# linkedin/spark-tfrecord

Measured on AMD Instinct MI355X. Metric: rows/sec read+write (1M-row Example round-trip), higher is better.
Workload: dtype wire(int64/float32/bytes); 1 GPU; model=Example{id:int64, ints:Int64List[8], floats:FloatList[16], tokens:BytesList[2]}, global_batch=1000000, parallelism=dp1, rows_per_rank=1000000, engine=gpu, storage=/dev/shm, crc_verify=True

## Files before the change

csrc/hip/kernels.hip:

```cpp

#include <hip/hip_runtime.h>
#include <pybind11/pybind11.h>
#include <pybind11/stl.h>
#include <rocprim/rocprim.hpp>

#include <fcntl.h>
#include <sys/mman.h>
#include <sys/stat.h>
#include <unistd.h>

#include <cstdint>
#include <map>
#include <mutex>
#include <stdexcept>
#include <string>
#include <vector>

#include "../codec_core.h"

namespace py = pybind11;
using namespace tfrec;

#define HIP_CHECK(expr)                                                          \
  do {                                                                           \
// ... 68 lines not shown
        rc = scan_record(data, off[r], len[r], fmt, schema, st);
        payload_crc = crc32c_sw(data + off[r], (size_t)len[r], 0, tab);
      }
      if (rc != ERR_OK)
        payload_crc = crc32c_sw(data + off[r], (size_t)len[r], 0, tab);
      const u8* h = data + off[r] - 12;
      u32 len_crc, data_crc;
      __builtin_memcpy(&len_crc, h + 8, 4);
      __builtin_memcpy(&data_crc, h + 12 + len[r], 4);
      bool ok = mask_crc(crc32c_sw(h, 8, 0, tab)) == len_crc &&
                mask_crc(payload_crc) == data_crc;
      if (!ok) atomicMin(crc_err, (unsigned long long)(rec_base + r + 1));
    } else {
      rc = scan_record(data, off[r], len[r], fmt, schema, st);
    }
    if (rc != ERR_OK) set_err(err, rc, rec_base + r);
    for (int f = 0; f < F; ++f)
      if (st[f].err != ERR_OK) set_err(err, st[f].err, rec_base + r);
  }
}


struct DevFieldDst {
  int32_t kind;
  int32_t is_seq;
  i64* i64_vals;
  float* f32_vals;
  u8* bytes_data;
  i64* elem_len;
  i64* sub_count;
  const i64* val_base;
  const i64* byte_base;
  const i64* list_base;
};

__global__ void extract_fields_kernel(const u8* __restrict__ data, i64 R, int F,
                                      const FieldStat* __restrict__ stats,
                                      const DevFieldDst* __restrict__ metas,
                                      int32_t* __restrict__ err, i64 r0) {
  i64 total = R * F;
  for (i64 idx = blockIdx.x * (i64)blockDim.x + threadIdx.x; idx < total;
       idx += (i64)gridDim.x * blockDim.x) {
    i64 q = idx / F;
    int f = (int)(idx - q * F);
    i64 r = r0 + q;
    const DevFieldDst& m = metas[f];
    const FieldStat& st = stats[r * F + f];
    DecodeDst dst{m.i64_vals, m.f32_vals, m.bytes_data, m.elem_len, m.sub_count};
    int32_t rc = extract_field(data, st.pos, st.len, m.kind, m.is_seq, dst,
                               m.val_base ? m.val_base[r] : 0,
                               m.byte_base ? m.byte_base[r] : 0,
                               m.list_base ? m.list_base[r] : 0);
    if (rc != ERR_OK) set_err(err, rc, r);
  }
}



__global__ void size_records_kernel(const FieldColumn* __restrict__ cols,
                                    const u8* __restrict__ schema_blob, int32_t fmt,
                                    i64 R, i64* __restrict__ psize) {
  SchemaView schema = schema_view(schema_blob);
  for (i64 r = blockIdx.x * (i64)blockDim.x + threadIdx.x; r < R;
       r += (i64)gridDim.x * blockDim.x) {
    psize[r] = record_payload_size(cols, schema, fmt, r) + kFrameOverhead;
  }
}

__global__ void emit_records_kernel(const FieldColumn* __restrict__ cols,
                                    const u8* __restrict__ schema_blob, int32_t fmt,
                                    i64 r0, i64 R, const i64* __restrict__ frame_off,
                                    u8* __restrict__ file,
                                    int32_t* __restrict__ err) {
  __shared__ uint32_t tab[8][256];
  stage_crc_tables(tab);
  SchemaView schema = schema_view(schema_blob);
  for (i64 r = r0 + blockIdx.x * (i64)blockDim.x + threadIdx.x; r < R;
       r += (i64)gridDim.x * blockDim.x) {
    i64 payload = (frame_off[r + 1] - frame_off[r]) - kFrameOverhead;
    u8* o = file + frame_off[r] + 12;
// ... 289 lines not shown
      if (rc != ERR_OK) set_err(err, rc, rec_base + r);
      for (int f = 0; f < F; ++f)
        if (st[f].err != ERR_OK) set_err(err, st[f].err, rec_base + r);
    }
    if (crc_err) {
      const u8* h = data + off[r] - 12;
      u32 payload = crc32c_wave(h + 12, len[r], tab);
      if (lane == 0) {
        u32 len_crc, data_crc;
        __builtin_memcpy(&len_crc, h + 8, 4);
        __builtin_memcpy(&data_crc, h + 12 + len[r], 4);
        bool ok = mask_crc(crc32c_sw(h, 8, 0, tab)) == len_crc &&
                  mask_crc(payload) == data_crc;
        if (!ok) atomicMin(crc_err, (unsigned long long)(rec_base + r + 1));
      }
    }
  }
}

__global__ void extract_fields_wave_kernel(const u8* __restrict__ data, i64 R,
                                           int F,
                                           const FieldStat* __restrict__ stats,
                                           const DevFieldDst* __restrict__ metas,
                                           int32_t* __restrict__ err, i64 r0) {
  i64 total = R * F;
  i64 wave = (blockIdx.x * (i64)blockDim.x + threadIdx.x) / 64;
  i64 nwaves = ((i64)gridDim.x * blockDim.x) / 64;
  for (i64 idx = wave; idx < total; idx += nwaves) {
    i64 q = idx / F;
    int f = (int)(idx - q * F);
    i64 r = r0 + q;
    const DevFieldDst& m = metas[f];
    const FieldStat& st = stats[r * F + f];
    DecodeDst dst{m.i64_vals, m.f32_vals, m.bytes_data, m.elem_len, m.sub_count};
    int32_t rc = extract_field_wave(data, st.pos, st.len, m.kind, m.is_seq, dst,
                                    m.val_base ? m.val_base[r] : 0,
                                    m.byte_base ? m.byte_base[r] : 0,
                                    m.list_base ? m.list_base[r] : 0);
    if (rc != ERR_OK && (threadIdx.x & 63) == 0) set_err(err, rc, r);
  }
}


__device__ inline i64 wave_emit_i64_packed(u8* __restrict__ o,
                                           const i64* __restrict__ vals,
                                           i64 v0, i64 v1) {
  int lane = threadIdx.x & 63;
  i64 n = v1 - v0;
  i64 chunk = (n + 63) / 64;
  i64 lo = v0 + (i64)lane * chunk;
  i64 hi = lo + chunk < v1 ? lo + chunk : v1;
  i64 sz = 0;
  for (i64 v = lo; v < hi; ++v) sz += varint_size((u64)vals[v]);
  i64 incl = wave_incl_scan(sz);
  u8* q = o + (incl - sz);
  for (i64 v = lo; v < hi; ++v) q = write_varint(q, (u64)vals[v]);
  return __shfl(incl, 63);
}

struct WaveCur {
  u8* base;
  i64 pos;
};

__device__ inline void wvc_put(WaveCur& w, u8 b) {
  if ((threadIdx.x & 63) == 0) w.base[w.pos] = b;
// ... 251 lines not shown
    }
    if (threadIdx.x == 0) block_data[block_base + blockIdx.x] = (i64)cnt[0];
    return;
  }
  for (int off = 1; off < (int)blockDim.x; off <<= 1) {
    unsigned int v = (int)threadIdx.x >= off ? cnt[threadIdx.x - off] : 0;
    __syncthreads();
    cnt[threadIdx.x] += v;
    __syncthreads();
  }
  i64 slot = block_data[block_base + blockIdx.x] + (i64)(cnt[threadIdx.x] - my);
  if (c < c_hi)
    eval_frame_chunk(data, wdata, N, c, pos_start, pos_end, tab,
                     [&](i64 i, i64 len) {
                       cand_pos[slot] = i;
                       cand_len[slot] = len;
                       ++slot;
                     });
}

__global__ void frame_chain_kernel(const i64* __restrict__ pos,
                                   const i64* __restrict__ len, i64 C,
                                   const i64* __restrict__ carry_in,
                                   i64* __restrict__ carry_out,
                                   i64* __restrict__ off,
                                   i64* __restrict__ broken) {
  for (i64 k = blockIdx.x * (i64)blockDim.x + threadIdx.x; k < C;
       k += (i64)gridDim.x * blockDim.x) {
    i64 p = pos[k];
    i64 want = k == 0 ? *carry_in : pos[k - 1] + 16 + len[k - 1];
    if (p != want) *broken = 1;
    off[k] = p + 12;
    if (k == C - 1) *carry_out = p + 16 + len[k];
  }
}


struct InferSlot {
  unsigned long long hash;
  long long nameref;
  long long code;
};
static_assert(sizeof(InferSlot) == 24, "layout shared with Python [S,3] i64");

__device__ inline u64 fnv1a64(const u8* s, u64 n) {
  u64 h = 1469598103934665603ull;
  for (u64 i = 0; i < n; ++i) h = (h ^ s[i]) * 1099511628211ull;
  return h ? h : 1ull;
}

constexpr int kLdsInfer = 64;

struct LdsInferSlot {
  unsigned long long hash;
  long long nameref;
  unsigned int code;
};

__device__ inline bool lds_infer_merge(LdsInferSlot* ltab, u64 hash,
                                       long long nameref, int code) {
  int idx = (int)(hash % (u64)kLdsInfer);
  for (int probe = 0; probe < kLdsInfer; ++probe) {
    LdsInferSlot& s = ltab[idx];
    unsigned long long seen =
        atomicCAS(&s.hash, 0ull, (unsigned long long)hash);
    if (seen == 0ull) s.nameref = nameref;
// ... 220 lines not shown
                       dim3(kBlock), 0, (hipStream_t)stream, (const u8*)data,
                       (const i64*)off, (const i64*)len, R,
                       (unsigned long long*)err_out);
  } else {
    hipLaunchKernelGGL(crc_verify_kernel, dim3(grid_for(R)), dim3(kBlock), 0,
                       (hipStream_t)stream, (const u8*)data, (const i64*)off,
                       (const i64*)len, R, (unsigned long long*)err_out);
  }
  HIP_CHECK(hipGetLastError());
}

void gpu_scan_records(uintptr_t data, uintptr_t off, uintptr_t len, i64 R,
                      int32_t fmt, uintptr_t schema_blob, int F, uintptr_t stats,
                      uintptr_t err, uintptr_t crc_err, uintptr_t stream,
                      i64 avg_bytes, i64 rec_base, i64 max_blocks) {
  if (R <= 0) return;
  if (avg_bytes > kWaveRecordBytes) {
    hipLaunchKernelGGL(scan_records_wave_kernel,
                       dim3(grid_for(R * 64, max_blocks)), dim3(kBlock), 0,
                       (hipStream_t)stream, (const u8*)data, (const i64*)off,
                       (const i64*)len, R, fmt, (const u8*)schema_blob, F,
                       (FieldStat*)stats, (int32_t*)err,
                       (unsigned long long*)crc_err, rec_base);
  } else {
    hipLaunchKernelGGL(scan_records_kernel, dim3(grid_for(R, max_blocks)),
                       dim3(kBlock), 0, (hipStream_t)stream, (const u8*)data,
                       (const i64*)off, (const i64*)len, R, fmt,
                       (const u8*)schema_blob, F, (FieldStat*)stats,
                       (int32_t*)err, (unsigned long long*)crc_err, rec_base);
  }
  HIP_CHECK(hipGetLastError());
}

void gpu_extract_fields(uintptr_t data, i64 R, int F, uintptr_t stats,
                        py::list metas, uintptr_t meta_dev, uintptr_t err,
                        uintptr_t stream, i64 avg_bytes, i64 r0,
                        i64 max_blocks) {
  if (R <= 0 || F <= 0) return;
  std::vector<DevFieldDst> host_metas(F);
  for (int f = 0; f < F; ++f) {
    py::dict d = metas[f].cast<py::dict>();
    DevFieldDst& m = host_metas[f];
    m.kind = d["kind"].cast<int32_t>();
    m.is_seq = d["is_seq"].cast<int32_t>();
    m.i64_vals = (i64*)d["i64_vals"].cast<uintptr_t>();
    m.f32_vals = (float*)d["f32_vals"].cast<uintptr_t>();
    m.bytes_data = (u8*)d["bytes_data"].cast<uintptr_t>();
    m.elem_len = (i64*)d["elem_len"].cast<uintptr_t>();
    m.sub_count = (i64*)d["sub_count"].cast<uintptr_t>();
    m.val_base = (const i64*)d["val_base"].cast<uintptr_t>();
    m.byte_base = (const i64*)d["byte_base"].cast<uintptr_t>();
    m.list_base = (const i64*)d["list_base"].cast<uintptr_t>();
  }
  HIP_CHECK(hipMemcpyAsync((void*)meta_dev, host_metas.data(),
                           sizeof(DevFieldDst) * F, hipMemcpyHostToDevice,
                           (hipStream_t)stream));
  if (avg_bytes > kWaveRecordBytes) {
    hipLaunchKernelGGL(extract_fields_wave_kernel,
                       dim3(grid_for(R * F * 64, max_blocks)), dim3(kBlock), 0,
                       (hipStream_t)stream, (const u8*)data, R, F,
                       (const FieldStat*)stats, (const DevFieldDst*)meta_dev,
                       (int32_t*)err, r0);
  } else {
    hipLaunchKernelGGL(extract_fields_kernel,
                       dim3(grid_for(R * F, max_blocks)), dim3(kBlock), 0,
                       (hipStream_t)stream, (const u8*)data, R, F,
                       (const FieldStat*)stats, (const DevFieldDst*)meta_dev,
                       (int32_t*)err, r0);
  }
  HIP_CHECK(hipGetLastError());
}

size_t gpu_devcols_bytes(int F) { return sizeof(FieldColumn) * (size_t)F; }

void fill_devcols(py::list cols, std::vector<FieldColumn>& out) {
  int F = (int)cols.size();
  out.resize(F);
  for (int f = 0; f < F; ++f) {
    py::dict d = cols[f].cast<py::dict>();
    FieldColumn& c = out[f];
    c.kind = d["kind"].cast<int32_t>();
    c.is_seq = d["is_seq"].cast<int32_t>();
    c.presence = (const u8*)d["presence"].cast<uintptr_t>();
    c.row_off = (const i64*)d["row_off"].cast<uintptr_t>();
    c.list_off = (const i64*)d["list_off"].cast<uintptr_t>();
    c.sub_off = (const i64*)d["sub_off"].cast<uintptr_t>();
    c.elem_off = (const i64*)d["elem_off"].cast<uintptr_t>();
    c.bytes_data = (const u8*)d["values_bytes"].cast<uintptr_t>();
    c.i64_vals = (const i64*)d["values_i64"].cast<uintptr_t>();
// ... 58 lines not shown
void gpu_frame_scan_count(uintptr_t data, i64 N, i64 pos_start, i64 pos_end,
                          i64 block_base, uintptr_t block_counts,
                          uintptr_t stream) {
  i64 B = gpu_frame_scan_blocks(pos_start, pos_end);
  if (B <= 0) return;
  hipLaunchKernelGGL(frame_scan_pass_kernel<false>, dim3((uint32_t)B),
                     dim3(kBlock), 0, (hipStream_t)stream, (const u8*)data, N,
                     pos_start, pos_end, block_base, (i64*)block_counts,
                     nullptr, nullptr);
  HIP_CHECK(hipGetLastError());
}

void gpu_frame_scan_emit(uintptr_t data, i64 N, i64 pos_start, i64 pos_end,
                         i64 block_base, uintptr_t block_off,
                         uintptr_t cand_pos, uintptr_t cand_len,
                         uintptr_t stream) {
  i64 B = gpu_frame_scan_blocks(pos_start, pos_end);
  if (B <= 0) return;
  hipLaunchKernelGGL(frame_scan_pass_kernel<true>, dim3((uint32_t)B),
                     dim3(kBlock), 0, (hipStream_t)stream, (const u8*)data, N,
                     pos_start, pos_end, block_base, (i64*)block_off,
                     (i64*)cand_pos, (i64*)cand_len);
  HIP_CHECK(hipGetLastError());
}

void gpu_frame_chain(uintptr_t pos, uintptr_t len, i64 C, uintptr_t carry_in,
                     uintptr_t carry_out, uintptr_t off, uintptr_t broken,
                     uintptr_t stream) {
  if (C <= 0) return;
  hipLaunchKernelGGL(frame_chain_kernel, dim3(grid_for(C)), dim3(kBlock), 0,
                     (hipStream_t)stream, (const i64*)pos, (const i64*)len, C,
                     (const i64*)carry_in, (i64*)carry_out, (i64*)off,
                     (i64*)broken);
  HIP_CHECK(hipGetLastError());
}

void gpu_infer_codes(uintptr_t data, uintptr_t off, uintptr_t len, i64 R,
                     int32_t fmt, uintptr_t table, int nslots, uintptr_t err,
                     uintptr_t stream) {
  hipLaunchKernelGGL(infer_codes_kernel, dim3(grid_for(R)), dim3(kBlock), 0,
                     (hipStream_t)stream, (const u8*)data, (const i64*)off,
                     (const i64*)len, R, fmt, (InferSlot*)table, nslots,
                     (int32_t*)err);
  HIP_CHECK(hipGetLastError());
}

void gpu_gather_payloads(uintptr_t data, uintptr_t off, uintptr_t len,
                         uintptr_t dst_off, i64 R, uintptr_t out,
                         uintptr_t stream, i64 avg_bytes) {
  if (avg_bytes > kWaveRecordBytes) {
    hipLaunchKernelGGL(gather_payloads_wave_kernel, dim3(grid_for(R * 64)),
                       dim3(kBlock), 0, (hipStream_t)stream, (const u8*)data,
                       (const i64*)off, (const i64*)len, (const i64*)dst_off,
                       R, (u8*)out);
  } else {
    hipLaunchKernelGGL(gather_payloads_kernel, dim3(grid_for(R)), dim3(kBlock),
                       0, (hipStream_t)stream, (const u8*)data,
                       (const i64*)off, (const i64*)len, (const i64*)dst_off,
                       R, (u8*)out);
  }
  HIP_CHECK(hipGetLastError());
}


struct StridedLoadI64 {
  const i64* p;
// ... 252 lines not shown


void gpu_memcpy_d2h(uintptr_t dst, uintptr_t src, i64 n, uintptr_t stream) {
  HIP_CHECK(hipMemcpyAsync((void*)dst, (const void*)src, (size_t)n,
                           hipMemcpyDeviceToHost, (hipStream_t)stream));
}

void gpu_memcpy_h2d(uintptr_t dst, uintptr_t src, i64 n, uintptr_t stream) {
  HIP_CHECK(hipMemcpyAsync((void*)dst, (const void*)src, (size_t)n,
                           hipMemcpyHostToDevice, (hipStream_t)stream));
}

}

void register_gpu(py::module_& m) {
  m.def("gpu_device_count", []() {
    int n = 0;
    hipError_t e = hipGetDeviceCount(&n);
    return (e == hipSuccess) ? n : -static_cast<int>(e);
  });
  m.def("gpu_crc_verify", &gpu_crc_verify, py::arg("data"), py::arg("off"),
        py::arg("len"), py::arg("R"), py::arg("err_out"), py::arg("stream"),
        py::arg("avg_bytes") = 0);
  m.def("gpu_scan_records", &gpu_scan_records, py::arg("data"), py::arg("off"),
        py::arg("len"), py::arg("R"), py::arg("fmt"), py::arg("schema_blob"),
        py::arg("F"), py::arg("stats"), py::arg("err"), py::arg("crc_err"),
        py::arg("stream"), py::arg("avg_bytes") = 0, py::arg("rec_base") = 0,
        py::arg("max_blocks") = 0);
  m.def("gpu_extract_fields", &gpu_extract_fields, py::arg("data"),
        py::arg("R"), py::arg("F"), py::arg("stats"), py::arg("metas"),
        py::arg("meta_dev"), py::arg("err"), py::arg("stream"),
        py::arg("avg_bytes") = 0, py::arg("r0") = 0,
        py::arg("max_blocks") = 0);
  m.def("gpu_size_records", &gpu_size_records);
  m.def("gpu_emit_records", &gpu_emit_records, py::arg("cols_dev"),
        py::arg("schema_blob"), py::arg("fmt"), py::arg("r0"), py::arg("R"),
        py::arg("frame_off"), py::arg("file"), py::arg("err"),
        py::arg("stream"), py::arg("avg_bytes") = 0);
  m.def("gpu_frame_bytes", &gpu_frame_bytes, py::arg("src"),
        py::arg("elem_off"), py::arg("frame_off"), py::arg("R"),
        py::arg("file"), py::arg("stream"), py::arg("avg_bytes") = 0);
  m.def("gpu_frame_scan_blocks", &gpu_frame_scan_blocks);
  m.def("gpu_frame_scan_count", &gpu_frame_scan_count);
  m.def("gpu_frame_scan_emit", &gpu_frame_scan_emit);
  m.def("gpu_frame_chain", &gpu_frame_chain);
  m.def("gpu_gather_payloads", &gpu_gather_payloads, py::arg("data"),
        py::arg("off"), py::arg("len"), py::arg("dst_off"), py::arg("R"),
        py::arg("out"), py::arg("stream"), py::arg("avg_bytes") = 0);
  m.def("gpu_infer_codes", &gpu_infer_codes);
  m.def("gpu_scan_temp_bytes", &gpu_scan_temp_bytes);
  m.def("gpu_stat_scan_temp_bytes", &gpu_stat_scan_temp_bytes);
  m.def("gpu_stat_scans", &gpu_stat_scans, py::arg("temp"),
        py::arg("temp_bytes"), py::arg("stats"), py::arg("R"), py::arg("F"),
        py::arg("val_base"), py::arg("byte_base"), py::arg("list_base"),
        py::arg("stream"), py::arg("r0") = 0, py::arg("r1") = -1,
        py::arg("stride") = 0);
  m.def("gpu_excl_sum_strided", &gpu_excl_sum_strided);
  m.def("file_mmap_pinned", &file_mmap_pinned, py::arg("path"), py::arg("n"),
        py::arg("writable"));
  m.def("file_mmap_drop", &file_mmap_drop);
  m.def("file_mmap_sync", &file_mmap_sync);
  m.def("gpu_memcpy_d2h", &gpu_memcpy_d2h);
  m.def("gpu_memcpy_h2d", &gpu_memcpy_h2d);
  m.def("gpu_devcols_bytes", &gpu_devcols_bytes);
  m.def("gpu_devmeta_bytes", []() { return sizeof(DevFieldDst); });
  m.def("gpu_fieldstat_words", []() { return sizeof(FieldStat) / 8; });
}
```

spark_tfrecord_amd/engine/gpu.py:

```python

from __future__ import annotations

import os
from typing import List, Optional

import numpy as np
import torch

from .. import _native
from . import stream_plan
from ..columnar import RecordBatch, WireColumn, schema_blob, wire_fields
from ..schema import KIND_BYTES, KIND_FLOAT, KIND_INT64, StructType, is_sequence_field, wire_kind_of

FMT = {"Example": _native.FMT_EXAMPLE, "SequenceExample": _native.FMT_SEQUENCE}

_U64_MAX = 0xFFFFFFFFFFFFFFFF


def _stream() -> int:
    return torch.cuda.current_stream().cuda_stream


def _dev(x, dtype, device="cuda") -> torch.Tensor:
    if isinstance(x, torch.Tensor):
# ... 8 lines not shown

def check_native():
    if not getattr(_native, "HAS_GPU_KERNELS", False):
        raise RuntimeError("_native was built without HIP kernels; rebuild "
                           "with build_native.py before using the GPU engine")



import threading as _threading

_pinned_tls = _threading.local()


def pinned_buffer(tag: str, nbytes: int) -> torch.Tensor:
    pool = getattr(_pinned_tls, "pool", None)
    if pool is None:
        pool = _pinned_tls.pool = {}
    buf = pool.get(tag)
    if buf is None or buf.numel() < nbytes:
        cap = max(nbytes, int((buf.numel() if buf is not None else 1 << 20) * 1.5))
        buf = torch.empty(cap, dtype=torch.uint8, pin_memory=True)
        pool[tag] = buf
    return buf


_CHUNK = 64 << 20
_READ_SLICE = int(os.environ.get("TFREC_READ_SLICE", 32 << 20))
_SPLIT_SLICES = os.environ.get("TFREC_READ_SPLIT", "1") != "0"
_WRITE_SLICES = int(os.environ.get("TFREC_WRITE_SLICES", 8))
_STREAM_DECODE = os.environ.get("TFREC_STREAM_DECODE", "1") != "0"
_STREAM_HEADROOM = float(os.environ.get("TFREC_STREAM_HEADROOM", 1.125))
_STREAM_MAX_BLOCKS = int(os.environ.get("TFREC_STREAM_MAX_BLOCKS", 0))
_STREAM_EXTRACT = os.environ.get("TFREC_STREAM_EXTRACT", "1") != "0"
_SYNC_WRITES = os.environ.get("TFREC_SYNC", "1") != "0"


def read_file_to_device(path: str, device="cuda") -> torch.Tensor:
    import os as _os

    n = _os.path.getsize(path)
    dev_t = torch.empty(max(n, 1), dtype=torch.uint8, device=device)[:n]
    if n:
        ptr, pinned = _native.file_mmap_pinned(path, n, False)
        if pinned:
            _multi_dma(dev_t.data_ptr(), ptr, n, _native.gpu_memcpy_h2d,
                       after_main=True)
            return dev_t
    return _read_file_staged(path, dev_t)


_copy_streams: Optional[list] = None


def _dma_streams() -> list:
    global _copy_streams
    if _copy_streams is None:
        _copy_streams = [torch.cuda.Stream() for _ in range(2)]
    return _copy_streams


def _multi_dma(dst: int, src: int, n: int, fn, after_main: bool):
    streams = _dma_streams()
    main = torch.cuda.current_stream()
    k = min(len(streams), max(1, n // (16 << 20)))
    span = (n + k - 1) // k
    for i in range(k):
# ... 524 lines not shown
    data = torch.empty(n, dtype=torch.uint8, device=device)
    device = data.device
    plan = stream_plan.plan_slices(n, _READ_SLICE)
    S = len(plan)
    nblocks = [int(_native.gpu_frame_scan_blocks(p.scan_lo, p.scan_hi))
               if p.scan_hi > p.scan_lo else 0 for p in plan]
    block_counts = torch.empty(max(sum(nblocks), 1), dtype=torch.int64,
                               device=device)
    main = torch.cuda.current_stream()
    streams = _dma_streams()
    events = []
    for st in streams:
        st.wait_stream(main)
    for s, p in enumerate(plan):
        half = (p.b1 - p.b0) // 2 if _SPLIT_SLICES and len(streams) > 1 else 0
        parts = ([(p.b0, p.b0 + half, 0), (p.b0 + half, p.b1, 1)] if half
                 else [(p.b0, p.b1, s % len(streams))])
        evs = []
        for lo, hi, k in parts:
            st = streams[k]
            _native.gpu_memcpy_h2d(data.data_ptr() + lo, ptr + lo, hi - lo,
                                   st.cuda_stream)
            ev = torch.cuda.Event()
            ev.record(st)
            evs.append(ev)
        events.append(evs)
    data.record_stream(streams[0])
    if len(streams) > 1:
        data.record_stream(streams[1])

    fields = wire_fields(schema)
    F = len(fields)
    streaming = _STREAM_DECODE
    last_read.update(path="streamed", slices=S, regrows=0)
    do_scan = streaming and record_type != "ByteArray" and F > 0
    fuse_crc = verify_crc
    vals = None
    if streaming:
        status = torch.zeros(_ST_CARRY + 1 + S, dtype=torch.int64,
                             device=device)
        status[_ST_CRC] = -1
        sp = status.data_ptr()
        err = status[_ST_ERR:_ST_ERR + 1].view(torch.int32)
        xerr = status[_ST_XERR:_ST_XERR + 1].view(torch.int32)
        rows = _StreamRows(n, F if do_scan else 0, device)
        if do_scan:
            blob = _schema_blob_device(schema, device)
            vals = _StreamValues(fields, n, device) if _STREAM_EXTRACT else None
            meta_dev = torch.empty(F * _native.gpu_devmeta_bytes(),
                                   dtype=torch.uint8, device=device)

    base = 0
    C = 0
    nchain = 0
    r_done = 0
    pending = None
    avg_bytes = None
    for s, p in enumerate(plan):
        for ev in events[s]:
            main.wait_event(ev)
        last = s == S - 1
        nb = nblocks[s]
        if nb:
            _native.gpu_frame_scan_count(data.data_ptr(), n, p.scan_lo,
                                         p.scan_hi, base,
                                         block_counts.data_ptr(), _stream())
        if not streaming:
            base += nb
            continue
        if nb:
            block_off = excl_sum(block_counts[base:base + nb])
            c_s = int(block_off[-1].item())
            base += nb
            if c_s:
                rows.reserve(C + c_s, C, r_done, p.scan_hi)
                _native.gpu_frame_scan_emit(
                    data.data_ptr(), n, p.scan_lo, p.scan_hi, 0,
                    block_off.data_ptr(), rows.pos.data_ptr() + C * 8,
                    rows.lens.data_ptr() + C * 8, _stream())
                _native.gpu_frame_chain(
                    rows.pos.data_ptr() + C * 8, rows.lens.data_ptr() + C * 8,
                    c_s, sp + (_ST_CARRY + nchain) * 8,
                    sp + (_ST_CARRY + 1 + nchain) * 8,
                    rows.off.data_ptr() + C * 8, sp + _ST_BROKEN * 8, _stream())
                nchain += 1
                C += c_s
        if not do_scan or C == r_done:
            continue
        if last:
            avail = C
            end = n
        else:
            st_h = status.cpu()
            if int(st_h[_ST_BROKEN]) != 0:
                streaming = do_scan = False
                continue
            end = int(st_h[_ST_CARRY + nchain])
            avail = stream_plan.arrived_records(C, end, p.b1)
            if avail < C:
                end = p.b1
        if avail > r_done:
            if avg_bytes is None:
                avg_bytes = max(0, end // avail - 16)
            _native.gpu_scan_records(
                data.data_ptr(), rows.off.data_ptr() + r_done * 8,
                rows.lens.data_ptr() + r_done * 8, avail - r_done,
                FMT[record_type], blob.data_ptr(), F,
                rows.stats.data_ptr() + r_done * F * 48, err.data_ptr(),
                sp + _ST_CRC * 8 if fuse_crc else 0, _stream(), avg_bytes,
                rec_base=r_done, max_blocks=0 if last else _STREAM_MAX_BLOCKS)
            if vals is not None:
                rows.scan_stats(r_done, avail)
                if last:
                    pending = (r_done, avail)
                elif vals.ok:
                    h = torch.cat(rows.totals(avail)
                                  + [status[:_ST_CARRY]]).cpu()
                    pair = h[3 * F + _ST_ERR:3 * F + _ST_ERR + 1].view(torch.int32)
                    if int(h[3 * F + _ST_CRC]) != -1 or int(pair[0]) != 0:
                        vals.ok = False
                    else:
                        vals.extract(data, rows, r_done, avail,
                                     h[:3 * F].view(3, F), end, meta_dev,
                                     xerr, avg_bytes,
                                     _STREAM_MAX_BLOCKS)
            r_done = avail

    def unstreamed():
        last_read["path"] = "fallback" if _STREAM_DECODE else "unstreamed"
        ranges = [(p.scan_lo, p.scan_hi) for p in plan if p.scan_hi > p.scan_lo]
        off, lens, _ = _emit_and_chain(data, ranges, block_counts, n)
        return decode_device(data, off, lens, schema, record_type, verify_crc)

    if not streaming or C == 0:
        return unstreamed()
    R = C
    if not do_scan:
        st_h = status.cpu()
        if int(st_h[_ST_BROKEN]) != 0 or int(st_h[_ST_CARRY + nchain]) != n:
            return unstreamed()
        return decode_device(data, rows.off[:R], rows.lens[:R], schema,
                             record_type, verify_crc)

    stats = rows.stats[:R]
    if vals is None:
        rows.scan_stats(0, R)
    packed = torch.cat(rows.totals(R) + [status]).cpu()
    st_h = packed[3 * F:]
    if int(st_h[_ST_BROKEN]) != 0 or int(st_h[_ST_CARRY + nchain]) != n:
        return unstreamed()
    pair = st_h[_ST_ERR:_ST_ERR + 1].view(torch.int32)
    _raise_scan_errors(int(st_h[_ST_CRC]) if fuse_crc else -1, int(pair[0]),
                       int(pair[1]))
    totals_h = packed[:3 * F].view(3, F)
    val_base, byte_base, list_base = rows.planes
    if vals is None:
        cols = _extract_columns(data, R, fields, stats,
                                val_base[:, :R + 1], byte_base[:, :R + 1],
                                list_base[:, :R + 1], totals_h, xerr,
                                max(0, n // R - 16))
    else:
        if not vals.ok:
            raise RuntimeError("streamed decode: scan error lost")
        if pending is not None:
            vals.extract(data, rows, pending[0], pending[1], totals_h, n,
                         meta_dev, xerr, avg_bytes, 0)
        cols = vals.columns(stats, val_base, list_base, R)
    err_h = xerr.cpu()
    if int(err_h[0]) != 0:
        _raise_extract_error(int(err_h[0]), int(err_h[1]))
    return RecordBatch(schema, cols, R)


_ST_BROKEN, _ST_CRC, _ST_ERR, _ST_XERR, _ST_CARRY = 0, 1, 2, 3, 4


class _StreamRows:

    def __init__(self, total_bytes: int, F: int, device):
        self.total_bytes = total_bytes
        self.F = F
        self.device = device
        self.cap = 0
        self.pos = self.lens = self.off = self.stats = None
        self.planes = None

    def _alloc(self, cap: int):
        i64 = dict(dtype=torch.int64, device=self.device)
        planes = None
        if self.F:
            planes = [torch.empty((self.F, cap + 1), **i64) for _ in range(3)]
            for t in planes:
                t[:, 0] = 0
        return (torch.empty(cap, **i64), torch.empty(cap, **i64),
                torch.empty(cap, **i64),
                torch.empty((cap, self.F, 6), **i64) if self.F else None,
                planes)

    def scan_stats(self, r0: int, r1: int):
        ws = _stat_scan_workspace(r1 - r0, self.F, self.device)
        v, b, l = self.planes
        _native.gpu_stat_scans(ws.data_ptr(), ws.numel(),
                               self.stats.data_ptr(), r1, self.F, v.data_ptr(),
                               b.data_ptr(), l.data_ptr(), _stream(), r0=r0,
                               r1=r1, stride=self.cap + 1)

    def totals(self, r: int) -> list:
        return [t[:, r] for t in self.planes]

    def reserve(self, need: int, n_cand: int, n_scanned: int, bytes_seen: int):
        cap = stream_plan.grown_capacity(self.cap, need, bytes_seen,
                                         self.total_bytes, _STREAM_HEADROOM)
        if cap == self.cap:
            return
        pos, lens, off, stats, planes = self._alloc(cap)
        if n_cand:
            pos[:n_cand].copy_(self.pos[:n_cand])
            lens[:n_cand].copy_(self.lens[:n_cand])
            off[:n_cand].copy_(self.off[:n_cand])
        if n_scanned and stats is not None:
            stats[:n_scanned].copy_(self.stats[:n_scanned])
            for new, old in zip(planes, self.planes):
                new[:, :n_scanned + 1].copy_(old[:, :n_scanned + 1])
        self.pos, self.lens, self.off, self.stats = pos, lens, off, stats
        self.planes = planes
        if self.cap:
            last_read["regrows"] = last_read.get("regrows", 0) + 1
        self.cap = cap


class _StreamValues:

    _DIMS = (("i64_vals", 0), ("f32_vals", 0), ("elem_len", 0),
             ("bytes_data", 1), ("sub_count", 2))

    def __init__(self, fields, total_bytes: int, device):
        self.total_bytes = total_bytes
        self.device = device
        self.ok = True
        self.kinds = [wire_kind_of(f.dataType) for f in fields]
        self.seqs = [is_sequence_field(f.dataType) for f in fields]
        self.filled = [[0] * len(fields) for _ in range(3)]
        self.bufs = []
        for kind in self.kinds:
            dt = {"i64_vals": torch.int64, "f32_vals": torch.float32,
                  "elem_len": torch.int64, "bytes_data": torch.uint8,
                  "sub_count": torch.int64}
            self.bufs.append({k: torch.empty(0, dtype=d, device=device)
                              for k, d in dt.items()})

    def _used(self, i: int, name: str) -> bool:
        kind = self.kinds[i]
        return {"i64_vals": kind == KIND_INT64, "f32_vals": kind == KIND_FLOAT,
                "elem_len": kind == KIND_BYTES}.get(name, True)

    def _reserve(self, totals, bytes_seen: int):
        for i, bufs in enumerate(self.bufs):
            for name, dim in self._DIMS:
                if not self._used(i, name):
                    continue
                need = int(totals[dim][i])
                old = bufs[name]
                cap = stream_plan.grown_capacity(
                    old.numel(), need, bytes_seen, self.total_bytes,
                    _STREAM_HEADROOM, min_unit=1)
                if cap == old.numel():
                    continue
                new = torch.empty(cap, dtype=old.dtype, device=self.device)
                k = self.filled[dim][i]
                if k:
                    new[:k].copy_(old[:k])
                if old.numel():
                    last_read["regrows"] = last_read.get("regrows", 0) + 1
                bufs[name] = new

    def extract(self, data, rows, r0: int, r1: int, totals, bytes_seen: int,
                meta_dev, xerr, avg_bytes: int, max_blocks: int):
        self._reserve(totals, bytes_seen)
        v, b, l = rows.planes
        metas = []
        for i, bufs in enumerate(self.bufs):
            metas.append({
                "kind": self.kinds[i], "is_seq": 1 if self.seqs[i] else 0,
                "i64_vals": bufs["i64_vals"].data_ptr(),
                "f32_vals": bufs["f32_vals"].data_ptr(),
                "bytes_data": bufs["bytes_data"].data_ptr(),
                "elem_len": bufs["elem_len"].data_ptr(),
                "sub_count": bufs["sub_count"].data_ptr(),
                "val_base": v[i].data_ptr(),
                "byte_base": b[i].data_ptr(),
                "list_base": l[i].data_ptr() if self.seqs[i] else 0,
            })
        _native.gpu_extract_fields(data.data_ptr(), r1 - r0, len(self.bufs),
                                   rows.stats.data_ptr(), metas,
                                   meta_dev.data_ptr(), xerr.data_ptr(),
                                   _stream(), avg_bytes, r0=r0,
                                   max_blocks=max_blocks)
        self.filled = [[int(totals[d][i]) for i in range(len(self.bufs))]
                       for d in range(3)]

    def columns(self, stats, val_base, list_base, R: int) -> List[WireColumn]:
        cols = []
        for i, bufs in enumerate(self.bufs):
            kind, seq = self.kinds[i], self.seqs[i]
            nv, nb, nl = (self.filled[d][i] for d in range(3))
            presence = (stats[:, i, 0] >= 0).to(torch.uint8)
            elem_off = None
            if kind == KIND_BYTES:
                elem_off = excl_sum(bufs["elem_len"][:nv])
            sub_off = None
            if seq:
                sub_off = excl_sum(bufs["sub_count"][:nl])
            values = (bufs["i64_vals"][:nv] if kind == KIND_INT64 else
                      bufs["f32_vals"][:nv] if kind == KIND_FLOAT else
                      bufs["bytes_data"][:nb])
            cols.append(WireColumn(kind, seq, presence, val_base[i][:R + 1],
                                   values, elem_off,
                                   list_base[i][:R + 1] if seq else None,
                                   sub_off))
        return cols


def gz_device_meta(path: str):
    from ..io import paths as P

    if not getattr(_native, "HAS_GPU_KERNELS", False):
        return None
    return P.parse_gz_segments_file(path)


def _device_inflate_group(data: torch.Tensor, gz_items, device) -> bool:
    import os as _os

    comp_sizes = [_os.path.getsize(p) for p, _, _ in gz_items]
    comp_total = sum(comp_sizes)
    comp = torch.empty(max(comp_total, 1), dtype=torch.uint8,
                       device=device)[:comp_total]
    main = torch.cuda.current_stream()
    streams = _dma_streams()
    in_off = []
    in_len = []
    out_off = []
    out_len = []
    used = []
    coff = 0
    for k, (p, meta, out_base) in enumerate(gz_items):
        body_off, segs, _crc, _isize = meta
        ptr, pinned = _native.file_mmap_pinned(p, comp_sizes[k], False)
        if pinned:
            st = streams[k % len(streams)]
# ... 324 lines not shown
```

spark_tfrecord_amd/engine/stream_plan.py:

```python

from __future__ import annotations

from typing import List, NamedTuple

MIN_FRAME = 16
SCAN_LOOKAHEAD = 32


class SlicePlan(NamedTuple):
    b0: int
    b1: int
    scan_lo: int
    scan_hi: int


def plan_slices(n: int, span: int) -> List[SlicePlan]:
    if n <= 0:
        return []
    span = max(1, int(span))
    S = (n + span - 1) // span
    out = []
    scanned = 0
    for s in range(S):
        b0, b1 = s * span, min(n, (s + 1) * span)
        hi = b1 - SCAN_LOOKAHEAD if s < S - 1 else n
        hi = max(hi, scanned)
        out.append(SlicePlan(b0, b1, scanned, hi))
        scanned = hi
    return out


def arrived_records(n_cand: int, last_end: int, arrived: int) -> int:
    if n_cand <= 0:
        return 0
    return n_cand if last_end <= arrived else n_cand - 1


def row_capacity(need: int, bytes_seen: int, total_bytes: int,
                 headroom: float, min_unit: int = MIN_FRAME) -> int:
    need = max(int(need), 0)
    bytes_seen = min(max(int(bytes_seen), 1), max(int(total_bytes), 1))
    est = int(need * (total_bytes / bytes_seen) * max(headroom, 1.0)) + 1
    most = need + max(total_bytes - bytes_seen, 0) // max(min_unit, 1)
    return max(need, min(est, most), 1)


def grown_capacity(cap: int, need: int, bytes_seen: int, total_bytes: int,
                   headroom: float, min_unit: int = MIN_FRAME) -> int:
    if need <= cap:
        return cap
    return row_capacity(need, bytes_seen, total_bytes, headroom, min_unit)
```

Measured before the change: 113.6 million rows/s.

## Pace streamed frame discovery on device and fold presence into field extraction

Adds a device-side frame discovery path (coarse count, emit with in-block prefix, chain kernel) that keeps the running candidate count and carry in a device status buffer. This removes the per-slice host readback of block-count prefix sums, leaving one status copy per slice, and falls back to the host-paced path on overflow. Presence bytes are now written inside the extract kernels instead of computed per column afterwards, and the field-destination metadata upload is skipped when unchanged. The cost is three launches per slice, redundant CRC frame evaluation (each chunk is evaluated three times), and an extra presence buffer to copy on regrow.

```diff
diff --git a/csrc/hip/kernels.hip b/csrc/hip/kernels.hip
--- a/csrc/hip/kernels.hip
+++ b/csrc/hip/kernels.hip
@@ -124,6 +124,7 @@
   const i64* val_base;
   const i64* byte_base;
   const i64* list_base;
+  u8* presence;
 };
 
 __global__ void extract_fields_kernel(const u8* __restrict__ data, i64 R, int F,
@@ -138,6 +139,7 @@
     i64 r = r0 + q;
     const DevFieldDst& m = metas[f];
     const FieldStat& st = stats[r * F + f];
+    if (m.presence) m.presence[r] = st.pos >= 0 ? 1 : 0;
     DecodeDst dst{m.i64_vals, m.f32_vals, m.bytes_data, m.elem_len, m.sub_count};
     int32_t rc = extract_field(data, st.pos, st.len, m.kind, m.is_seq, dst,
                                m.val_base ? m.val_base[r] : 0,
@@ -493,6 +495,8 @@
     i64 r = r0 + q;
     const DevFieldDst& m = metas[f];
     const FieldStat& st = stats[r * F + f];
+    if (m.presence && (threadIdx.x & 63) == 0)
+      m.presence[r] = st.pos >= 0 ? 1 : 0;
     DecodeDst dst{m.i64_vals, m.f32_vals, m.bytes_data, m.elem_len, m.sub_count};
     int32_t rc = extract_field_wave(data, st.pos, st.len, m.kind, m.is_seq, dst,
                                     m.val_base ? m.val_base[r] : 0,
@@ -810,6 +814,160 @@
     if (p != want) *broken = 1;
     off[k] = p + 12;
     if (k == C - 1) *carry_out = p + 16 + len[k];
+  }
+}
+
+constexpr int kCoarseMaxIters = 16;
+constexpr int kFlagBroken = 0;
+constexpr int kFlagOverflow = 4;
+
+__global__ void frame_count_coarse_kernel(const u8* __restrict__ data, i64 N,
+                                          i64 pos_start, i64 pos_end, int iters,
+                                          i64* __restrict__ counts) {
+  __shared__ uint32_t tab[8][256];
+  __shared__ unsigned int cnt[kBlock];
+  stage_crc_tables(tab);
+  const u64* wdata = reinterpret_cast<const u64*>(data);
+  i64 c_hi = (pos_end + kPosPerLane - 1) / kPosPerLane;
+  i64 cb = pos_start / kPosPerLane + (i64)blockIdx.x * blockDim.x * iters;
+  unsigned int my = 0;
+  for (int j = 0; j < iters; ++j) {
+    i64 c = cb + (i64)j * blockDim.x + threadIdx.x;
+    if (c < c_hi)
+      eval_frame_chunk(data, wdata, N, c, pos_start, pos_end, tab,
+                       [&](i64, i64) { ++my; });
+  }
+  cnt[threadIdx.x] = my;
+  __syncthreads();
+  for (int off = blockDim.x / 2; off; off >>= 1) {
+    if ((int)threadIdx.x < off) cnt[threadIdx.x] += cnt[threadIdx.x + off];
+    __syncthreads();
+  }
+  if (threadIdx.x == 0) counts[blockIdx.x] = (i64)cnt[0];
+}
+
+__device__ inline void coarse_count_sums(const i64* __restrict__ counts, i64 nb,
+                                         i64 upto, i64 (*red)[kBlock],
+                                         i64* pre, i64* total) {
+  i64 p = 0, t = 0;
+  for (i64 k = threadIdx.x; k < nb; k += blockDim.x) {
+    i64 v = counts[k];
+    t += v;
+    if (k < upto) p += v;
+  }
+  red[0][threadIdx.x] = p;
+  red[1][threadIdx.x] = t;
+  __syncthreads();
+  for (int off = blockDim.x / 2; off; off >>= 1) {
+    if ((int)threadIdx.x < off) {
+      red[0][threadIdx.x] += red[0][threadIdx.x + off];
+      red[1][threadIdx.x] += red[1][threadIdx.x + off];
+    }
+    __syncthreads();
+  }
+  *pre = red[0][0];
+  *total = red[1][0];
+}
+
+__global__ void frame_emit_coarse_kernel(const u8* __restrict__ data, i64 N,
+                                         i64 pos_start, i64 pos_end, int iters,
+                                         const i64* __restrict__ counts, i64 nb,
+                                         const i64* __restrict__ cum_in,
+                                         const i64* __restrict__ flags, i64 cap,
+                                         i64* __restrict__ cand_pos,
+                                         i64* __restrict__ cand_len) {
+  __shared__ uint32_t tab[8][256];
+  __shared__ unsigned int cnt[kCoarseMaxIters * kBlock];
+  __shared__ unsigned int sums[kBlock];
+  __shared__ i64 red[2][kBlock];
+  stage_crc_tables(tab);
+  i64 pre, total;
+  coarse_count_sums(counts, nb, blockIdx.x, red, &pre, &total);
+  i64 C0 = *cum_in;
+  if (flags[kFlagOverflow] != 0) return;
+  if (C0 < 0 || C0 + total > cap) return;
+  const u64* wdata = reinterpret_cast<const u64*>(data);
+  i64 c_hi = (pos_end + kPosPerLane - 1) / kPosPerLane;
+  i64 cb = pos_start / kPosPerLane + (i64)blockIdx.x * blockDim.x * iters;
+  for (int j = 0; j < iters; ++j) {
+    i64 c = cb + (i64)j * blockDim.x + threadIdx.x;
+    unsigned int my = 0;
+    if (c < c_hi)
+      eval_frame_chunk(data, wdata, N, c, pos_start, pos_end, tab,
+                       [&](i64, i64) { ++my; });
+    cnt[j * blockDim.x + threadIdx.x] = my;
+  }
+  __syncthreads();
+  unsigned int s = 0;
+  for (int i = 0; i < iters; ++i) s += cnt[threadIdx.x * iters + i];
+  sums[threadIdx.x] = s;
+  __syncthreads();
+  for (int off = 1; off < (int)blockDim.x; off <<= 1) {
+    unsigned int v = (int)threadIdx.x >= off ? sums[threadIdx.x - off] : 0;
+    __syncthreads();
+    sums[threadIdx.x] += v;
+    __syncthreads();
+  }
+  unsigned int e = sums[threadIdx.x] - s;
+  for (int i = 0; i < iters; ++i) {
+    unsigned int v = cnt[threadIdx.x * iters + i];
+    cnt[threadIdx.x * iters + i] = e;
+    e += v;
+  }
+  __syncthreads();
+  for (int j = 0; j < iters; ++j) {
+    i64 c = cb + (i64)j * blockDim.x + threadIdx.x;
+    if (c >= c_hi) continue;
+    i64 slot = C0 + pre + (i64)cnt[j * blockDim.x + threadIdx.x];
+    eval_frame_chunk(data, wdata, N, c, pos_start, pos_end, tab,
+                     [&](i64 i, i64 len) {
+                       if (slot < cap) {
+                         cand_pos[slot] = i;
+                         cand_len[slot] = len;
+                       }
+                       ++slot;
+                     });
+  }
+}
+
+__global__ void frame_chain_dev_kernel(const i64* __restrict__ pos,
+                                       const i64* __restrict__ len,
+                                       const i64* __restrict__ counts, i64 nb,
+                                       i64 cap, i64 slice,
+                                       const i64* __restrict__ cum_in,
+                                       i64* __restrict__ cum_out,
+                                       const i64* __restrict__ carry_in,
+                                       i64* __restrict__ carry_out,
+                                       i64* __restrict__ off,
+                                       i64* __restrict__ flags) {
+  __shared__ i64 red[2][kBlock];
+  i64 pre, total;
+  coarse_count_sums(counts, nb, 0, red, &pre, &total);
+  i64 C0 = *cum_in;
+  bool first = blockIdx.x == 0 && threadIdx.x == 0;
+  if (flags[kFlagOverflow] != 0) return;
+  if (C0 < 0 || C0 + total > cap) {
+    if (first) flags[kFlagOverflow] = slice + 1;
+    return;
+  }
+  if (total == 0) {
+    if (first) {
+      *cum_out = C0;
+      *carry_out = *carry_in;
+    }
+    return;
+  }
+  for (i64 k = blockIdx.x * (i64)blockDim.x + threadIdx.x; k < total;
+       k += (i64)gridDim.x * blockDim.x) {
+    i64 g = C0 + k;
+    i64 p = pos[g];
+    i64 want = k == 0 ? *carry_in : pos[g - 1] + 16 + len[g - 1];
+    if (p != want) flags[kFlagBroken] = 1;
+    off[g] = p + 12;
+    if (k == total - 1) {
+      *carry_out = p + 16 + len[g];
+      *cum_out = C0 + total;
+    }
   }
 }
 
@@ -1096,11 +1254,10 @@
   HIP_CHECK(hipGetLastError());
 }
 
-void gpu_extract_fields(uintptr_t data, i64 R, int F, uintptr_t stats,
-                        py::list metas, uintptr_t meta_dev, uintptr_t err,
-                        uintptr_t stream, i64 avg_bytes, i64 r0,
-                        i64 max_blocks) {
-  if (R <= 0 || F <= 0) return;
+void gpu_upload_field_dst(py::list metas, uintptr_t meta_dev,
+                          uintptr_t stream) {
+  int F = (int)py::len(metas);
+  if (F <= 0) return;
   std::vector<DevFieldDst> host_metas(F);
   for (int f = 0; f < F; ++f) {
     py::dict d = metas[f].cast<py::dict>();
@@ -1115,10 +1272,25 @@
     m.val_base = (const i64*)d["val_base"].cast<uintptr_t>();
     m.byte_base = (const i64*)d["byte_base"].cast<uintptr_t>();
     m.list_base = (const i64*)d["list_base"].cast<uintptr_t>();
+    m.presence = d.contains("presence")
+                     ? (u8*)d["presence"].cast<uintptr_t>() : nullptr;
   }
   HIP_CHECK(hipMemcpyAsync((void*)meta_dev, host_metas.data(),
                            sizeof(DevFieldDst) * F, hipMemcpyHostToDevice,
                            (hipStream_t)stream));
+}
+
+void gpu_extract_fields(uintptr_t data, i64 R, int F, uintptr_t stats,
+                        py::object metas, uintptr_t meta_dev, uintptr_t err,
+                        uintptr_t stream, i64 avg_bytes, i64 r0,
+                        i64 max_blocks) {
+  if (R <= 0 || F <= 0) return;
+  if (!metas.is_none()) {
+    py::list lst = metas.cast<py::list>();
+    if ((int)py::len(lst) != F)
+      throw std::runtime_error("gpu_extract_fields: metas length != F");
+    gpu_upload_field_dst(lst, meta_dev, stream);
+  }
   if (avg_bytes > kWaveRecordBytes) {
     hipLaunchKernelGGL(extract_fields_wave_kernel,
                        dim3(grid_for(R * F * 64, max_blocks)), dim3(kBlock), 0,
@@ -1243,6 +1415,45 @@
                      (hipStream_t)stream, (const i64*)pos, (const i64*)len, C,
                      (const i64*)carry_in, (i64*)carry_out, (i64*)off,
                      (i64*)broken);
+  HIP_CHECK(hipGetLastError());
+}
+
+i64 gpu_frame_coarse_blocks(i64 pos_start, i64 pos_end, int iters) {
+  if (iters < 1 || iters > kCoarseMaxIters)
+    throw std::runtime_error("frame discovery: iters outside [1, 16]");
+  i64 c_lo = pos_start / kPosPerLane;
+  i64 c_hi = (pos_end + kPosPerLane - 1) / kPosPerLane;
+  i64 per = (i64)kBlock * iters;
+  return (c_hi - c_lo + per - 1) / per;
+}
+
+void gpu_frame_discover_dev(uintptr_t data, i64 N, i64 pos_start, i64 pos_end,
+                            int iters, uintptr_t counts, i64 counts_cap,
+                            uintptr_t pos, uintptr_t len, uintptr_t off,
+                            i64 cap, i64 slice, uintptr_t status, i64 cum_in,
+                            i64 cum_out, i64 carry_in, i64 carry_out,
+                            i64 chain_budget, uintptr_t stream) {
+  i64 B = gpu_frame_coarse_blocks(pos_start, pos_end, iters);
+  if (B <= 0) return;
+  if (B > counts_cap || B > 0x7FFFFFFF)
+    throw std::runtime_error("frame discovery: count buffer too small");
+  if (cum_in == cum_out || carry_in == carry_out)
+    throw std::runtime_error("frame discovery: in/out words alias");
+  auto s = (hipStream_t)stream;
+  i64* st = (i64*)status;
+  hipLaunchKernelGGL(frame_count_coarse_kernel, dim3((uint32_t)B),
+                     dim3(kBlock), 0, s, (const u8*)data, N, pos_start,
+                     pos_end, iters, (i64*)counts);
+  hipLaunchKernelGGL(frame_emit_coarse_kernel, dim3((uint32_t)B), dim3(kBlock),
+                     0, s, (const u8*)data, N, pos_start, pos_end, iters,
+                     (const i64*)counts, B, (const i64*)(st + cum_in),
+                     (const i64*)st, cap, (i64*)pos, (i64*)len);
+  hipLaunchKernelGGL(frame_chain_dev_kernel, dim3(grid_for(chain_budget)),
+                     dim3(kBlock), 0, s, (const i64*)pos, (const i64*)len,
+                     (const i64*)counts, B, cap, slice,
+                     (const i64*)(st + cum_in), st + cum_out,
+                     (const i64*)(st + carry_in), st + carry_out, (i64*)off,
+                     st);
   HIP_CHECK(hipGetLastError());
 }
 
@@ -1561,6 +1772,7 @@
         py::arg("meta_dev"), py::arg("err"), py::arg("stream"),
         py::arg("avg_bytes") = 0, py::arg("r0") = 0,
         py::arg("max_blocks") = 0);
+  m.def("gpu_upload_field_dst", &gpu_upload_field_dst);
   m.def("gpu_size_records", &gpu_size_records);
   m.def("gpu_emit_records", &gpu_emit_records, py::arg("cols_dev"),
         py::arg("schema_blob"), py::arg("fmt"), py::arg("r0"), py::arg("R"),
@@ -1573,6 +1785,14 @@
   m.def("gpu_frame_scan_count", &gpu_frame_scan_count);
   m.def("gpu_frame_scan_emit", &gpu_frame_scan_emit);
   m.def("gpu_frame_chain", &gpu_frame_chain);
+  m.def("gpu_frame_coarse_blocks", &gpu_frame_coarse_blocks);
+  m.def("gpu_frame_discover_dev", &gpu_frame_discover_dev, py::arg("data"),
+        py::arg("N"), py::arg("pos_start"), py::arg("pos_end"),
+        py::arg("iters"), py::arg("counts"), py::arg("counts_cap"),
+        py::arg("pos"), py::arg("len"), py::arg("off"), py::arg("cap"),
+        py::arg("slice"), py::arg("status"), py::arg("cum_in"),
+        py::arg("cum_out"), py::arg("carry_in"), py::arg("carry_out"),
+        py::arg("chain_budget"), py::arg("stream"));
   m.def("gpu_gather_payloads", &gpu_gather_payloads, py::arg("data"),
         py::arg("off"), py::arg("len"), py::arg("dst_off"), py::arg("R"),
         py::arg("out"), py::arg("stream"), py::arg("avg_bytes") = 0);
diff --git a/spark_tfrecord_amd/engine/gpu.py b/spark_tfrecord_amd/engine/gpu.py
--- a/spark_tfrecord_amd/engine/gpu.py
+++ b/spark_tfrecord_amd/engine/gpu.py
@@ -64,6 +64,8 @@
 _STREAM_HEADROOM = float(os.environ.get("TFREC_STREAM_HEADROOM", 1.125))
 _STREAM_MAX_BLOCKS = int(os.environ.get("TFREC_STREAM_MAX_BLOCKS", 0))
 _STREAM_EXTRACT = os.environ.get("TFREC_STREAM_EXTRACT", "1") != "0"
+_STREAM_DEVICE = os.environ.get("TFREC_STREAM_DEVICE", "1") != "0"
+_COARSE_ITERS = int(os.environ.get("TFREC_COUNT_ROUNDS", 8))
 _SYNC_WRITES = os.environ.get("TFREC_SYNC", "1") != "0"
 
 
@@ -654,12 +656,13 @@
     fields = wire_fields(schema)
     F = len(fields)
     streaming = _STREAM_DECODE
-    last_read.update(path="streamed", slices=S, regrows=0)
+    last_read.update(path="streamed", slices=S, regrows=0, paced="host",
+                     host_syncs=0)
     do_scan = streaming and record_type != "ByteArray" and F > 0
     fuse_crc = verify_crc
     vals = None
     if streaming:
-        status = torch.zeros(_ST_CARRY + 1 + S, dtype=torch.int64,
+        status = torch.zeros(_ST_CARRY + 2 * (S + 1), dtype=torch.int64,
                              device=device)
         status[_ST_CRC] = -1
         sp = status.data_ptr()
@@ -672,6 +675,12 @@
             meta_dev = torch.empty(F * _native.gpu_devmeta_bytes(),
                                    dtype=torch.uint8, device=device)
 
+    dev_paced = streaming and do_scan and _STREAM_DEVICE
+    dev_used = False
+    cum0 = _ST_CARRY + S + 1
+    coarse = None
+    fine_counted = [False] * S
+    syncs = 0
     base = 0
     C = 0
     nchain = 0
@@ -683,16 +692,46 @@
             main.wait_event(ev)
         last = s == S - 1
         nb = nblocks[s]
-        if nb:
+        st_h = None
+        if nb and dev_paced and do_scan and C > 0:
+            nbc = int(_native.gpu_frame_coarse_blocks(p.scan_lo, p.scan_hi,
+                                                      _COARSE_ITERS))
+            if coarse is None or coarse.numel() < nbc:
+                coarse = torch.empty(nbc, dtype=torch.int64, device=device)
+            if not dev_used:
+                status[cum0 + nchain] = C
+                dev_used = True
+                last_read["paced"] = "device"
+            _native.gpu_frame_discover_dev(
+                data.data_ptr(), n, p.scan_lo, p.scan_hi, _COARSE_ITERS,
+                coarse.data_ptr(), coarse.numel(), rows.pos.data_ptr(),
+                rows.lens.data_ptr(), rows.off.data_ptr(), rows.cap, s, sp,
+                cum0 + nchain, cum0 + nchain + 1, _ST_CARRY + nchain,
+                _ST_CARRY + nchain + 1,
+                stream_plan.slice_budget(C, p.scan_lo, p.scan_hi - p.scan_lo,
+                                         _STREAM_HEADROOM), _stream())
+            st_h = status.cpu()
+            syncs += 1
+            if int(st_h[_ST_OVF]) != 0:
+                dev_paced = False
+                st_h = None
+                last_read["paced"] = f"device->host@{s}"
+            else:
+                nchain += 1
+                C = int(st_h[cum0 + nchain])
+                base += nb
+        if nb and st_h is None:
             _native.gpu_frame_scan_count(data.data_ptr(), n, p.scan_lo,
                                          p.scan_hi, base,
                                          block_counts.data_ptr(), _stream())
+            fine_counted[s] = True
         if not streaming:
             base += nb
             continue
-        if nb:
+        if nb and st_h is None:
             block_off = excl_sum(block_counts[base:base + nb])
             c_s = int(block_off[-1].item())
+            syncs += 1
             base += nb
             if c_s:
                 rows.reserve(C + c_s, C, r_done, p.scan_hi)
@@ -713,7 +752,9 @@
             avail = C
             end = n
         else:
-            st_h = status.cpu()
+            if st_h is None:
+                st_h = status.cpu()
+                syncs += 1
             if int(st_h[_ST_BROKEN]) != 0:
                 streaming = do_scan = False
                 continue
@@ -738,6 +779,7 @@
                 elif vals.ok:
                     h = torch.cat(rows.totals(avail)
                                   + [status[:_ST_CARRY]]).cpu()
+                    syncs += 1
                     pair = h[3 * F + _ST_ERR:3 * F + _ST_ERR + 1].view(torch.int32)
                     if int(h[3 * F + _ST_CRC]) != -1 or int(pair[0]) != 0:
                         vals.ok = False
@@ -750,6 +792,14 @@
 
     def unstreamed():
         last_read["path"] = "fallback" if _STREAM_DECODE else "unstreamed"
+        last_read["host_syncs"] = syncs
+        b = 0
+        for k, p in enumerate(plan):
+            if nblocks[k] and not fine_counted[k]:
+                _native.gpu_frame_scan_count(data.data_ptr(), n, p.scan_lo,
+                                             p.scan_hi, b,
+                                             block_counts.data_ptr(), _stream())
+            b += nblocks[k]
         ranges = [(p.scan_lo, p.scan_hi) for p in plan if p.scan_hi > p.scan_lo]
         off, lens, _ = _emit_and_chain(data, ranges, block_counts, n)
         return decode_device(data, off, lens, schema, record_type, verify_crc)
@@ -768,6 +818,7 @@
     if vals is None:
         rows.scan_stats(0, R)
     packed = torch.cat(rows.totals(R) + [status]).cpu()
+    last_read["host_syncs"] = syncs + 2
     st_h = packed[3 * F:]
     if int(st_h[_ST_BROKEN]) != 0 or int(st_h[_ST_CARRY + nchain]) != n:
         return unstreamed()
@@ -787,14 +838,14 @@
         if pending is not None:
             vals.extract(data, rows, pending[0], pending[1], totals_h, n,
                          meta_dev, xerr, avg_bytes, 0)
-        cols = vals.columns(stats, val_base, list_base, R)
+        cols = vals.columns(rows.presence, val_base, list_base, R)
     err_h = xerr.cpu()
     if int(err_h[0]) != 0:
         _raise_extract_error(int(err_h[0]), int(err_h[1]))
     return RecordBatch(schema, cols, R)
 
 
-_ST_BROKEN, _ST_CRC, _ST_ERR, _ST_XERR, _ST_CARRY = 0, 1, 2, 3, 4
+_ST_BROKEN, _ST_CRC, _ST_ERR, _ST_XERR, _ST_OVF, _ST_CARRY = 0, 1, 2, 3, 4, 5
 
 
 class _StreamRows:
@@ -805,6 +856,7 @@
         self.device = device
         self.cap = 0
         self.pos = self.lens = self.off = self.stats = None
+        self.presence = None
         self.planes = None
 
     def _alloc(self, cap: int):
@@ -817,7 +869,9 @@
         return (torch.empty(cap, **i64), torch.empty(cap, **i64),
                 torch.empty(cap, **i64),
                 torch.empty((cap, self.F, 6), **i64) if self.F else None,
-                planes)
+                planes,
+                torch.empty((self.F, cap), dtype=torch.uint8,
+                            device=self.device) if self.F else None)
 
     def scan_stats(self, r0: int, r1: int):
         ws = _stat_scan_workspace(r1 - r0, self.F, self.device)
@@ -835,7 +889,7 @@
                                          self.total_bytes, _STREAM_HEADROOM)
         if cap == self.cap:
             return
-        pos, lens, off, stats, planes = self._alloc(cap)
+        pos, lens, off, stats, planes, presence = self._alloc(cap)
         if n_cand:
             pos[:n_cand].copy_(self.pos[:n_cand])
             lens[:n_cand].copy_(self.lens[:n_cand])
@@ -844,8 +898,10 @@
             stats[:n_scanned].copy_(self.stats[:n_scanned])
             for new, old in zip(planes, self.planes):
                 new[:, :n_scanned + 1].copy_(old[:, :n_scanned + 1])
+            presence[:, :n_scanned].copy_(self.presence[:, :n_scanned])
         self.pos, self.lens, self.off, self.stats = pos, lens, off, stats
         self.planes = planes
+        self.presence = presence
         if self.cap:
             last_read["regrows"] = last_read.get("regrows", 0) + 1
         self.cap = cap
@@ -863,6 +919,7 @@
         self.kinds = [wire_kind_of(f.dataType) for f in fields]
         self.seqs = [is_sequence_field(f.dataType) for f in fields]
         self.filled = [[0] * len(fields) for _ in range(3)]
+        self._uploaded = None
         self.bufs = []
         for kind in self.kinds:
             dt = {"i64_vals": torch.int64, "f32_vals": torch.float32,
@@ -912,7 +969,13 @@
                 "val_base": v[i].data_ptr(),
                 "byte_base": b[i].data_ptr(),
                 "list_base": l[i].data_ptr() if self.seqs[i] else 0,
+                "presence": rows.presence[i].data_ptr(),
             })
+        key = (meta_dev.data_ptr(), metas)
+        if key == self._uploaded:
+            metas = None
+        else:
+            self._uploaded = key
         _native.gpu_extract_fields(data.data_ptr(), r1 - r0, len(self.bufs),
                                    rows.stats.data_ptr(), metas,
                                    meta_dev.data_ptr(), xerr.data_ptr(),
@@ -921,12 +984,11 @@
         self.filled = [[int(totals[d][i]) for i in range(len(self.bufs))]
                        for d in range(3)]
 
-    def columns(self, stats, val_base, list_base, R: int) -> List[WireColumn]:
+    def columns(self, presence, val_base, list_base, R: int) -> List[WireColumn]:
         cols = []
         for i, bufs in enumerate(self.bufs):
             kind, seq = self.kinds[i], self.seqs[i]
             nv, nb, nl = (self.filled[d][i] for d in range(3))
-            presence = (stats[:, i, 0] >= 0).to(torch.uint8)
             elem_off = None
             if kind == KIND_BYTES:
                 elem_off = excl_sum(bufs["elem_len"][:nv])
@@ -936,8 +998,8 @@
             values = (bufs["i64_vals"][:nv] if kind == KIND_INT64 else
                       bufs["f32_vals"][:nv] if kind == KIND_FLOAT else
                       bufs["bytes_data"][:nb])
-            cols.append(WireColumn(kind, seq, presence, val_base[i][:R + 1],
-                                   values, elem_off,
+            cols.append(WireColumn(kind, seq, presence[i][:R],
+                                   val_base[i][:R + 1], values, elem_off,
                                    list_base[i][:R + 1] if seq else None,
                                    sub_off))
         return cols
diff --git a/spark_tfrecord_amd/engine/stream_plan.py b/spark_tfrecord_amd/engine/stream_plan.py
--- a/spark_tfrecord_amd/engine/stream_plan.py
+++ b/spark_tfrecord_amd/engine/stream_plan.py
@@ -36,6 +36,17 @@
     return n_cand if last_end <= arrived else n_cand - 1
 
 
+def slice_budget(rows_seen: int, bytes_seen: int, slice_bytes: int,
+                 headroom: float) -> int:
+    slice_bytes = max(int(slice_bytes), 0)
+    most = slice_bytes // MIN_FRAME
+    bytes_seen = max(int(bytes_seen), 1)
+    rows_seen = max(int(rows_seen), 0)
+    floor = -(-rows_seen * slice_bytes // bytes_seen)
+    est = int(floor * max(headroom, 1.0)) + 1
+    return min(max(est, floor), most)
+
+
 def row_capacity(need: int, bytes_seen: int, total_bytes: int,
                  headroom: float, min_unit: int = MIN_FRAME) -> int:
     need = max(int(need), 0)
```

Result: no change. 115.0 million rows/s (median of 6 runs) (+1.3%).
